# lrjconan/LanczosNetwork

Measured on NVIDIA H100. Metric: QM8 molecules/sec (forward), higher is better.
Workload: dtype f32

## Files before the change

### lanczosnetwork_b200/csrc/sm90.cuh

```cuda
#pragma once
#include <cuda.h>
#include <cuda_runtime.h>
#include <stdint.h>

namespace sm90 {

__device__ __forceinline__ uint32_t smem_u32(const void* p) {
  return static_cast<uint32_t>(__cvta_generic_to_shared(p));
}

__device__ __forceinline__ void mbar_init(uint64_t* bar, uint32_t count) {
  asm volatile("mbarrier.init.shared::cta.b64 [%0], %1;" ::"r"(smem_u32(bar)), "r"(count));
}
__device__ __forceinline__ void fence_barrier_init() {
  asm volatile("fence.mbarrier_init.release.cluster;" ::: "memory");
}
__device__ __forceinline__ void mbar_arrive(uint64_t* bar) {
  asm volatile("mbarrier.arrive.shared::cta.b64 _, [%0];" ::"r"(smem_u32(bar)) : "memory");
}
__device__ __forceinline__ void mbar_arrive_expect_tx(uint64_t* bar, uint32_t bytes) {
  asm volatile("mbarrier.arrive.expect_tx.shared::cta.b64 _, [%0], %1;" ::"r"(smem_u32(bar)),
               "r"(bytes)
               : "memory");
}
__device__ __forceinline__ bool mbar_try_wait(uint64_t* bar, uint32_t parity) {
  uint32_t ok;
  asm volatile(
      "{\n\t.reg .pred p;\n\t"
      "mbarrier.try_wait.parity.shared::cta.b64 p, [%1], %2;\n\t"
      "selp.b32 %0, 1, 0, p;\n\t}"
      : "=r"(ok)
      : "r"(smem_u32(bar)), "r"(parity)
      : "memory");
  return ok != 0;
}
__device__ __forceinline__ void mbar_wait(uint64_t* bar, uint32_t parity) {
  while (!mbar_try_wait(bar, parity)) {
  }
}

__device__ __forceinline__ void tma_prefetch_desc(const CUtensorMap* m) {
  asm volatile("prefetch.tensormap [%0];" ::"l"(reinterpret_cast<uint64_t>(m)) : "memory");
}
__device__ __forceinline__ void tma_load_2d(void* smem_dst, const CUtensorMap* m, uint64_t* bar,
                                            int32_t c0, int32_t c1) {
  asm volatile(
      "cp.async.bulk.tensor.2d.shared::cluster.global.mbarrier::complete_tx::bytes"
      " [%0], [%1, {%3, %4}], [%2];"
      ::"r"(smem_u32(smem_dst)), "l"(reinterpret_cast<uint64_t>(m)), "r"(smem_u32(bar)), "r"(c0),
      "r"(c1)
      : "memory");
}

__device__ __forceinline__ void cp_async_16(void* smem_dst, const void* gmem_src) {
  asm volatile("cp.async.cg.shared.global [%0], [%1], 16;" ::"r"(smem_u32(smem_dst)), "l"(gmem_src)
               : "memory");
}
__device__ __forceinline__ void cp_async_4(void* smem_dst, const void* gmem_src) {
  asm volatile("cp.async.ca.shared.global [%0], [%1], 4;" ::"r"(smem_u32(smem_dst)), "l"(gmem_src)
               : "memory");
}
__device__ __forceinline__ void cp_async_wait_all() {
  asm volatile("cp.async.commit_group;\n\tcp.async.wait_group 0;" ::: "memory");
}

__device__ __forceinline__ void fence_proxy_async() {
  asm volatile("fence.proxy.async.shared::cta;" ::: "memory");
}

__device__ __forceinline__ bool elect_one() {
  uint32_t pred;
  asm volatile(
      "{\n\t.reg .pred p;\n\t"
      "elect.sync _|p, 0xffffffff;\n\t"
      "selp.b32 %0, 1, 0, p;\n\t}"
      : "=r"(pred));
  return pred != 0;
}

__device__ __forceinline__ uint32_t tf32_rna_bits(float v) {
  uint32_t r;
  asm("cvt.rna.tf32.f32 %0, %1;" : "=r"(r) : "f"(v));
  return r;
}

__device__ __forceinline__ uint64_t wgmma_desc_kmajor_sw128(uint32_t smem_addr) {
  uint64_t d = 0;
  d |= (uint64_t)((smem_addr >> 4) & 0x3FFFu);
  d |= (uint64_t)1 << 16;
  d |= (uint64_t)64 << 32;
  d |= (uint64_t)1 << 62;
  return d;
}
__device__ __forceinline__ void wgmma_fence() { asm volatile("wgmma.fence.sync.aligned;" ::: "memory"); }
__device__ __forceinline__ void wgmma_commit() { asm volatile("wgmma.commit_group.sync.aligned;" ::: "memory"); }
__device__ __forceinline__ void wgmma_wait_all() { asm volatile("wgmma.wait_group.sync.aligned 0;" ::: "memory"); }


__device__ __forceinline__ void wgmma_n128(float (&d)[128], uint64_t a_desc, uint64_t b_desc, uint32_t scale_d) {
  asm volatile(
      "{\n\t.reg .pred p;\n\t"
      "setp.ne.b32 p, %66, 0;\n\t"
      "wgmma.mma_async.sync.aligned.m64n128k8.f32.tf32.tf32 "
      "{"
      "%0, %1, %2, %3, %4, %5, %6, %7, %8, %9, %10, %11, %12, %13, %14, %15, "
      "%16, %17, %18, %19, %20, %21, %22, %23, %24, %25, %26, %27, %28, %29, %30, %31, "
      "%32, %33, %34, %35, %36, %37, %38, %39, %40, %41, %42, %43, %44, %45, %46, %47, "
      "%48, %49, %50, %51, %52, %53, %54, %55, %56, %57, %58, %59, %60, %61, %62, %63"
      "}, %64, %65, p, 1, 1;\n\t}"
      : "+f"(d[0]), "+f"(d[1]), "+f"(d[2]), "+f"(d[3]), "+f"(d[4]), "+f"(d[5]), "+f"(d[6]), "+f"(d[7]),
        "+f"(d[8]), "+f"(d[9]), "+f"(d[10]), "+f"(d[11]), "+f"(d[12]), "+f"(d[13]), "+f"(d[14]), "+f"(d[15]),
        "+f"(d[16]), "+f"(d[17]), "+f"(d[18]), "+f"(d[19]), "+f"(d[20]), "+f"(d[21]), "+f"(d[22]), "+f"(d[23]),
        "+f"(d[24]), "+f"(d[25]), "+f"(d[26]), "+f"(d[27]), "+f"(d[28]), "+f"(d[29]), "+f"(d[30]), "+f"(d[31]),
        "+f"(d[32]), "+f"(d[33]), "+f"(d[34]), "+f"(d[35]), "+f"(d[36]), "+f"(d[37]), "+f"(d[38]), "+f"(d[39]),
        "+f"(d[40]), "+f"(d[41]), "+f"(d[42]), "+f"(d[43]), "+f"(d[44]), "+f"(d[45]), "+f"(d[46]), "+f"(d[47]),
        "+f"(d[48]), "+f"(d[49]), "+f"(d[50]), "+f"(d[51]), "+f"(d[52]), "+f"(d[53]), "+f"(d[54]), "+f"(d[55]),
        "+f"(d[56]), "+f"(d[57]), "+f"(d[58]), "+f"(d[59]), "+f"(d[60]), "+f"(d[61]), "+f"(d[62]), "+f"(d[63])
      : "l"(a_desc), "l"(b_desc), "r"(scale_d));
}

__device__ __forceinline__ void wgmma_n128_hi(float (&d)[128], uint64_t a_desc, uint64_t b_desc, uint32_t scale_d) {
  asm volatile(
      "{\n\t.reg .pred p;\n\t"
      "setp.ne.b32 p, %66, 0;\n\t"
      "wgmma.mma_async.sync.aligned.m64n128k8.f32.tf32.tf32 "
      "{"
      "%0, %1, %2, %3, %4, %5, %6, %7, %8, %9, %10, %11, %12, %13, %14, %15, "
      "%16, %17, %18, %19, %20, %21, %22, %23, %24, %25, %26, %27, %28, %29, %30, %31, "
      "%32, %33, %34, %35, %36, %37, %38, %39, %40, %41, %42, %43, %44, %45, %46, %47, "
      "%48, %49, %50, %51, %52, %53, %54, %55, %56, %57, %58, %59, %60, %61, %62, %63"
      "}, %64, %65, p, 1, 1;\n\t}"
      : "+f"(d[64]), "+f"(d[65]), "+f"(d[66]), "+f"(d[67]), "+f"(d[68]), "+f"(d[69]), "+f"(d[70]), "+f"(d[71]),
        "+f"(d[72]), "+f"(d[73]), "+f"(d[74]), "+f"(d[75]), "+f"(d[76]), "+f"(d[77]), "+f"(d[78]), "+f"(d[79]),
        "+f"(d[80]), "+f"(d[81]), "+f"(d[82]), "+f"(d[83]), "+f"(d[84]), "+f"(d[85]), "+f"(d[86]), "+f"(d[87]),
        "+f"(d[88]), "+f"(d[89]), "+f"(d[90]), "+f"(d[91]), "+f"(d[92]), "+f"(d[93]), "+f"(d[94]), "+f"(d[95]),
        "+f"(d[96]), "+f"(d[97]), "+f"(d[98]), "+f"(d[99]), "+f"(d[100]), "+f"(d[101]), "+f"(d[102]), "+f"(d[103]),
        "+f"(d[104]), "+f"(d[105]), "+f"(d[106]), "+f"(d[107]), "+f"(d[108]), "+f"(d[109]), "+f"(d[110]), "+f"(d[111]),
        "+f"(d[112]), "+f"(d[113]), "+f"(d[114]), "+f"(d[115]), "+f"(d[116]), "+f"(d[117]), "+f"(d[118]), "+f"(d[119]),
        "+f"(d[120]), "+f"(d[121]), "+f"(d[122]), "+f"(d[123]), "+f"(d[124]), "+f"(d[125]), "+f"(d[126]), "+f"(d[127])
      : "l"(a_desc), "l"(b_desc), "r"(scale_d));
}

}
```

### lanczosnetwork_b200/csrc/tc_gemm.cuh

```cuda
#pragma once
#include "common.cuh"
#include "sm90.cuh"
#include <stdlib.h>
#include <type_traits>

namespace tcg {

constexpr int BM = 128, BN = 128, BK = 32;
constexpr int NGROUPS = 1;
constexpr int TILE_B_BYTES = BN * BK * 4;
constexpr int STAGE_B_BYTES = 2 * TILE_B_BYTES;
constexpr int TILE_A_BYTES = BM * BK * 4;
constexpr int STAGE_A_BYTES = 2 * TILE_A_BYTES;
constexpr int EW = 16;
constexpr int PRODUCER_THREADS = 128 * NGROUPS;
constexpr int CONSUMER_WARP0 = PRODUCER_THREADS / 32;
constexpr int CONSUMER_THREADS = 256;
constexpr int THREADS = PRODUCER_THREADS + CONSUMER_THREADS;
constexpr int MAX_B_STAGES = 6, MAX_A_STAGES = 4;
__host__ __device__ constexpr int core_smem(int stages_b, int stages_a) {
  return stages_b * STAGE_B_BYTES + stages_a * STAGE_A_BYTES + 256;
}
__host__ __device__ constexpr int pass_cols(int stages_a) {
  return stages_a * STAGE_A_BYTES / (BM * 4) < BN ? stages_a * STAGE_A_BYTES / (BM * 4) : BN;
}

__device__ __forceinline__ uint8_t* a_ring(uint8_t* policy_smem, int stages_b, int stages_a) {
  return policy_smem - core_smem(stages_b, stages_a) + stages_b * STAGE_B_BYTES;
}

struct Core {
  uint8_t* Bst;
  uint8_t* Ast;
  uint64_t* b_full;
  uint64_t* b_empty;
  uint64_t* a_full;
  uint64_t* a_empty;
  uint64_t* stg_full;
  uint64_t* stg_empty;
  uint64_t* kept_read;
};

__device__ __forceinline__ Core carve(uint8_t* base, int stages_b, int stages_a) {
  Core c;
  c.Bst = base;
  c.Ast = base + stages_b * STAGE_B_BYTES;
  uint64_t* bars = reinterpret_cast<uint64_t*>(c.Ast + stages_a * STAGE_A_BYTES);
  c.b_full = bars;
  c.b_empty = c.b_full + MAX_B_STAGES;
  c.a_full = c.b_empty + MAX_B_STAGES;
  c.a_empty = c.a_full + MAX_A_STAGES;
  c.stg_full = c.a_empty + MAX_A_STAGES;
  c.stg_empty = c.stg_full + 1;
  c.kept_read = c.stg_empty + 1;
  return c;
}

__device__ unsigned long long* g_prof = nullptr;

struct PhaseTimer {
  unsigned long long* buf;
  long long t0;
  __device__ __forceinline__ void start(int cta, int tid) {
    buf = (tid == 0 && g_prof) ? g_prof + cta * 32 : nullptr;
    if (buf) t0 = clock64();
  }
  __device__ __forceinline__ void start_if(int cta, bool owner) {
    buf = (owner && g_prof) ? g_prof + cta * 32 : nullptr;
    if (buf) t0 = clock64();
  }
  __device__ __forceinline__ void lap(int slot) {
    if (buf) { long long t = clock64(); atomicAdd(&buf[slot], (unsigned long long)(t - t0)); t0 = t; }
  }
};

__device__ __forceinline__ void producers_sync() {
  asm volatile("bar.sync 1, %0;" ::"n"(PRODUCER_THREADS) : "memory");
}
__device__ __forceinline__ void consumers_sync() {
  asm volatile("bar.sync 2, %0;" ::"n"(CONSUMER_THREADS) : "memory");
}

__device__ __forceinline__ int stg_index(int row, int col, int pw) {
  return row * pw + ((((col >> 2) ^ row) & (pw / 4 - 1)) << 2) + (col & 3);
}

template <class P, class = void> struct HasAccInit : std::false_type {};
template <class P> struct HasAccInit<P, std::void_t<decltype(&P::acc_init)>> : std::true_type {};
template <class P, class = void> struct HasOperandFromAcc : std::false_type {};
template <class P> struct HasOperandFromAcc<P, std::void_t<decltype(&P::operand_from_acc)>> : std::true_type {};

template <class Policy>
__device__ __forceinline__ bool next_from_acc(const typename Policy::Params& p, int cta, int ncta, int it,
                                              int nsteps, int& nkb_next) {
  if (it + 1 >= nsteps) return false;
  int m_tile, sub;
  Policy::decode(p, cta, ncta, it + 1, m_tile, sub);
  nkb_next = Policy::num_kblocks(p, sub);
  return Policy::operand_from_acc(p, sub);
}

template <class Policy>
__global__ void __launch_bounds__(THREADS, 1)
tc_gemm_kernel(const __grid_constant__ CUtensorMap map_hi,
               const __grid_constant__ CUtensorMap map_lo, const typename Policy::Params p) {
  extern __shared__ __align__(16) uint8_t smem_raw[];
  const uint32_t pad = (1024u - (sm90::smem_u32(smem_raw) & 1023u)) & 1023u;
  uint8_t* base = smem_raw + pad;
  constexpr int SB = Policy::kStagesB, SA = Policy::kStagesA;
  static_assert(SB >= 1 && SB <= MAX_B_STAGES && SA >= 1 && SA <= MAX_A_STAGES, "ring depths");
  constexpr int PW = pass_cols(SA);
  constexpr int NPASS = BN / PW;
  constexpr bool kAccInit = HasAccInit<Policy>::value;
  static_assert(!kAccInit || NPASS == 1, "a drain kept in the A ring must fit it in one pass");
  constexpr bool kOpAcc = HasOperandFromAcc<Policy>::value;
  static_assert(!kOpAcc || SA * BK >= BN, "an operand written from the accumulators needs one A stage per k-block");
  Core c = carve(base, SB, SA);
  uint8_t* policy_smem = base + core_smem(SB, SA);
  float* stg = reinterpret_cast<float*>(c.Ast);

  const int tid = threadIdx.x, warp = tid >> 5, lane = tid & 31;
  const int cta = blockIdx.x, ncta = gridDim.x;
  const int nsteps = Policy::num_steps(p, cta, ncta);
  unsigned long long prof_ns0 = 0;
  long long prof_c0 = 0;
  if (tid == 0 && g_prof) {
    asm volatile("mov.u64 %0, %globaltimer;" : "=l"(prof_ns0));
    prof_c0 = clock64();
  }

  if (warp == CONSUMER_WARP0 && lane == 0) {
    sm90::tma_prefetch_desc(&map_hi);
    sm90::tma_prefetch_desc(&map_lo);
    for (int s = 0; s < SB; ++s) {
      sm90::mbar_init(&c.b_full[s], 1);
      sm90::mbar_init(&c.b_empty[s], CONSUMER_THREADS / 32);
    }
    for (int s = 0; s < SA; ++s) {
      sm90::mbar_init(&c.a_full[s], PRODUCER_THREADS);
      sm90::mbar_init(&c.a_empty[s], CONSUMER_THREADS / 32);
    }
    sm90::mbar_init(c.stg_full, CONSUMER_THREADS);
    sm90::mbar_init(c.stg_empty, PRODUCER_THREADS);
    sm90::mbar_init(c.kept_read, CONSUMER_THREADS / 32);
    sm90::fence_barrier_init();
  }
  __syncthreads();

  if (warp < CONSUMER_WARP0) {
    const int r = tid & 127;
    Policy pol(p, policy_smem, tid);
    uint32_t cnt = 0;
    uint32_t npass = 0;
    uint32_t nkept = 0;
    bool after_kept = false;
    for (int it = 0; it < nsteps; ++it) {
      int m_tile, sub;
      Policy::decode(p, cta, ncta, it, m_tile, sub);
      int nkb = Policy::num_kblocks(p, sub);
      bool kept = false, to_acc = false;
      if constexpr (kAccInit) kept = Policy::drain_kept(p, sub);
      if constexpr (kOpAcc) {
        if (Policy::operand_from_acc(p, sub)) nkb = 0;
        int nkb_next;
        to_acc = next_from_acc<Policy>(p, cta, ncta, it, nsteps, nkb_next);
      }
      PhaseTimer tm;
      tm.start(cta, tid);
      pol.step_begin(m_tile, sub, 0, tm);
      for (int kb = 0; kb < nkb; ++kb, ++cnt) {
        float v[32];
        if (!(p.dbg & 8)) pol.produce(sub, kb, v);
        const uint32_t sa = cnt % SA;
        if (kAccInit && kb == 0 && after_kept) {
          sm90::mbar_wait(c.kept_read, nkept & 1u);
          ++nkept;
        }
        sm90::mbar_wait(&c.a_empty[sa], ((cnt / SA) & 1u) ^ 1u);
        if (!(p.dbg & 1)) {
          uint8_t* hi = c.Ast + sa * STAGE_A_BYTES + r * 128;
#pragma unroll
          for (int j = 0; j < 8; ++j) {
            uint4 h, l;
            h.x = sm90::tf32_rna_bits(v[4 * j + 0]); h.y = sm90::tf32_rna_bits(v[4 * j + 1]);
            h.z = sm90::tf32_rna_bits(v[4 * j + 2]); h.w = sm90::tf32_rna_bits(v[4 * j + 3]);
            l.x = sm90::tf32_rna_bits(v[4 * j + 0] - __uint_as_float(h.x));
            l.y = sm90::tf32_rna_bits(v[4 * j + 1] - __uint_as_float(h.y));
            l.z = sm90::tf32_rna_bits(v[4 * j + 2] - __uint_as_float(h.z));
            l.w = sm90::tf32_rna_bits(v[4 * j + 3] - __uint_as_float(h.w));
            const int off = (j ^ (r & 7)) * 16;
            *reinterpret_cast<uint4*>(hi + off) = h;
            *reinterpret_cast<uint4*>(hi + TILE_A_BYTES + off) = l;
          }
        }
        sm90::fence_proxy_async();
        sm90::mbar_arrive(&c.a_full[sa]);
      }
      tm.lap((sub & 1) ? 8 : 3);
      pol.pre_epilogue(sub);
      tm.lap(4);
#pragma unroll 1
      for (int q = 0; q < (kept || to_acc ? 0 : NPASS); ++q, ++npass) {
        sm90::mbar_wait(c.stg_full, npass & 1u);
        if (q == 0) tm.lap((sub & 1) ? 9 : 5);
#pragma unroll 1
        for (int col = q * PW; col < (q + 1) * PW; col += EW) {
          float x[EW];
#pragma unroll
          for (int j = 0; j < EW; j += 4) {
            const float4 t = *reinterpret_cast<const float4*>(stg + stg_index(r, col - q * PW + j, PW));
            x[j] = t.x; x[j + 1] = t.y; x[j + 2] = t.z; x[j + 3] = t.w;
          }
          pol.store(sub, col, x);
        }
        sm90::mbar_arrive(c.stg_empty);
      }
      tm.lap(7);
      producers_sync();
      pol.post_epilogue(sub);
      tm.lap(10);
      after_kept = kept;
    }
  } else {
    const int wg = (warp - CONSUMER_WARP0) >> 2;
    const int wq = warp & 3;
    float d[128];
    uint32_t cnt = 0, npass = 0;
    uint32_t nacc = 0;
    bool after_kept = false;
    const int row0 = wg * 64 + wq * 16 + (lane >> 2), cl = 2 * (lane & 3);
    const bool issuer = warp == CONSUMER_WARP0;
    int l_it = 0, l_kb = 0, l_nkb = -1, l_sub = 0;
    uint32_t l_cnt = 0;
    auto load_next = [&]() {
      while (l_it < nsteps) {
        if (l_nkb < 0) {
          int mt;
          Policy::decode(p, cta, ncta, l_it, mt, l_sub);
          l_nkb = Policy::num_kblocks(p, l_sub);
        }
        if (l_kb < l_nkb) break;
        ++l_it; l_kb = 0; l_nkb = -1;
      }
      if (l_it >= nsteps) return;
      int col0, row0;
      Policy::w_coords(p, l_sub, l_kb, col0, row0);
      const uint32_t st = l_cnt % SB;
      sm90::mbar_wait(&c.b_empty[st], ((l_cnt / SB) & 1u) ^ 1u);
      if (sm90::elect_one()) {
        if (p.dbg & 4) {
          sm90::mbar_arrive(&c.b_full[st]);
        } else {
          uint8_t* dst = c.Bst + st * STAGE_B_BYTES;
          sm90::mbar_arrive_expect_tx(&c.b_full[st], STAGE_B_BYTES);
          sm90::tma_load_2d(dst, &map_hi, &c.b_full[st], col0, row0);
          sm90::tma_load_2d(dst + TILE_B_BYTES, &map_lo, &c.b_full[st], col0, row0);
        }
      }
      __syncwarp();
      ++l_kb; ++l_cnt;
    };
    if (issuer)
      for (int i = 0; i < SB; ++i) load_next();
    for (int it = 0; it < nsteps; ++it) {
      int m_tile, sub;
      Policy::decode(p, cta, ncta, it, m_tile, sub);
      const int nkb = Policy::num_kblocks(p, sub);
      bool kept = false, from_acc = false, to_acc = false;
      int nkb_next = 0;
      if constexpr (kOpAcc) {
        from_acc = Policy::operand_from_acc(p, sub);
        to_acc = next_from_acc<Policy>(p, cta, ncta, it, nsteps, nkb_next);
      }
      if constexpr (kAccInit) {
        kept = Policy::drain_kept(p, sub);
        if (!Policy::acc_init(p, policy_smem, stg, sub, row0, cl, d)) {
#pragma unroll
          for (int i = 0; i < 128; ++i) d[i] = 0.f;
        }
        if (after_kept) {
          __syncwarp();
          if (lane == 0) sm90::mbar_arrive(c.kept_read);
        }
      } else {
#pragma unroll
        for (int i = 0; i < 128; ++i) d[i] = 0.f;
      }
      for (int kb = 0; kb < nkb; ++kb, ++cnt) {
        const uint32_t acnt = cnt - nacc;
        const uint32_t sb = cnt % SB, sa = from_acc ? (uint32_t)kb : acnt % SA;
        sm90::mbar_wait(&c.b_full[sb], (cnt / SB) & 1u);
        if (!from_acc) sm90::mbar_wait(&c.a_full[sa], (acnt / SA) & 1u);
        if (!(p.dbg & 2)) {
          const uint32_t a_hi = sm90::smem_u32(c.Ast + sa * STAGE_A_BYTES) + wg * 64 * 128;
          const uint32_t a_lo = a_hi + TILE_A_BYTES;
          const uint32_t b = sm90::smem_u32(c.Bst + sb * STAGE_B_BYTES);
          sm90::wgmma_fence();
#pragma unroll
          for (int k = 0; k < BK / 8; ++k) {
            const uint64_t ah = sm90::wgmma_desc_kmajor_sw128(a_hi + 32 * k);
            const uint64_t wh = sm90::wgmma_desc_kmajor_sw128(b + 32 * k);
            sm90::wgmma_n128(d, ah, wh, 1u);
            sm90::wgmma_n128_hi(d, ah, sm90::wgmma_desc_kmajor_sw128(b + TILE_B_BYTES + 32 * k), 1u);
            sm90::wgmma_n128_hi(d, sm90::wgmma_desc_kmajor_sw128(a_lo + 32 * k), wh, 1u);
          }
          sm90::wgmma_commit();
          sm90::wgmma_wait_all();
        }
        __syncwarp();
        if (lane == 0) {
          if (!from_acc) sm90::mbar_arrive(&c.a_empty[sa]);
          sm90::mbar_arrive(&c.b_empty[sb]);
        }
        if (issuer) load_next();
      }
      if (from_acc) nacc += nkb;
      PhaseTimer ctm;
      if (to_acc) ctm.start_if(cta, tid == PRODUCER_THREADS);
      consumers_sync();
      if (to_acc) {
        if constexpr (kOpAcc) {
#pragma unroll
          for (int i = 0; i < 64; i += 2) {
            const int col = 8 * (i / 4) + cl, row = row0 + 8 * ((i / 2) % 2), kb = i / 16;
            if (kb < nkb_next) {
              const float y0 = Policy::acc_operand(p, policy_smem, sub, col, d[i] + d[i + 64]);
              const float y1 = Policy::acc_operand(p, policy_smem, sub, col + 1, d[i + 1] + d[i + 65]);
              uint2 h, l;
              h.x = sm90::tf32_rna_bits(y0); h.y = sm90::tf32_rna_bits(y1);
              l.x = sm90::tf32_rna_bits(y0 - __uint_as_float(h.x));
              l.y = sm90::tf32_rna_bits(y1 - __uint_as_float(h.y));
              uint8_t* dst = c.Ast + kb * STAGE_A_BYTES + row * 128 + (((((col & 31) >> 2) ^ row) & 7) << 4) +
                             (col & 3) * 4;
              *reinterpret_cast<uint2*>(dst) = h;
              *reinterpret_cast<uint2*>(dst + TILE_A_BYTES) = l;
            }
          }
          sm90::fence_proxy_async();
          consumers_sync();
          ctm.lap(14);
        }
      } else {
#pragma unroll
        for (int q = 0; q < NPASS; ++q, npass += kept ? 0 : 1) {
          if (!kept) sm90::mbar_wait(c.stg_empty, (npass & 1u) ^ 1u);
#pragma unroll
          for (int i = 0; i < 64; i += 2) {
            const int col = 8 * (i / 4) + cl, row = row0 + 8 * ((i / 2) % 2);
            if (col >= q * PW && col < (q + 1) * PW)
              *reinterpret_cast<float2*>(stg + stg_index(row, col - q * PW, PW)) =
                  make_float2(d[i] + d[i + 64], d[i + 1] + d[i + 65]);
          }
          if (!kept) sm90::mbar_arrive(c.stg_full);
        }
      }
      if (kept) consumers_sync();
      after_kept = kept;
    }
  }

  __syncthreads();
  if (tid == 0 && g_prof) {
    unsigned long long ns1;
    asm volatile("mov.u64 %0, %globaltimer;" : "=l"(ns1));
    atomicAdd(&g_prof[cta * 32 + 11], ns1 - prof_ns0);
    atomicAdd(&g_prof[cta * 32 + 12], (unsigned long long)(clock64() - prof_c0));
    g_prof[cta * 32 + 13] = prof_ns0;
  }
}

__device__ __forceinline__ void store_row_chunk(float* orow, int ncols, const float* bias, bool relu,
                                                int col, const float (&x)[EW]) {
  if (orow == nullptr || col >= ncols) return;
  const bool vec_ok = (reinterpret_cast<uintptr_t>(orow + col) & 15) == 0;
#pragma unroll
  for (int j = 0; j < EW; j += 4) {
    float o[4];
#pragma unroll
    for (int u = 0; u < 4; ++u) {
      const int n = col + j + u;
      float y = x[j + u];
      if (n < ncols) {
        if (bias) y += __ldg(bias + n);
        if (relu) y = fmaxf(y, 0.f);
      }
      o[u] = y;
    }
    if (vec_ok && col + j + 3 < ncols) {
      *reinterpret_cast<float4*>(orow + col + j) = make_float4(o[0], o[1], o[2], o[3]);
    } else {
#pragma unroll
      for (int u = 0; u < 4; ++u)
        if (col + j + u < ncols) orow[col + j + u] = o[u];
    }
  }
}

typedef CUresult (*EncodeTiledFn)(CUtensorMap*, CUtensorMapDataType, cuuint32_t, void*,
                                  const cuuint64_t*, const cuuint64_t*, const cuuint32_t*,
                                  const cuuint32_t*, CUtensorMapInterleave, CUtensorMapSwizzle,
                                  CUtensorMapL2promotion, CUtensorMapFloatOOBfill);

inline EncodeTiledFn get_encode_fn() {
  static EncodeTiledFn fn = nullptr;
  if (!fn) {
    void* ptr = nullptr;
    cudaDriverEntryPointQueryResult q;
    if (cudaGetDriverEntryPoint("cuTensorMapEncodeTiled", &ptr, cudaEnableDefault, &q) == cudaSuccess &&
        q == cudaDriverEntryPointSuccess)
      fn = reinterpret_cast<EncodeTiledFn>(ptr);
  }
  return fn;
}

inline int make_weight_map(CUtensorMap* map, const float* W, int rows, int cols, const char* who,
                           int box_rows = BN) {
  EncodeTiledFn enc = get_encode_fn();
  if (!enc) { lnb::set_err("%s: cuTensorMapEncodeTiled unavailable", who); return LNB_ERR_UNSUPPORTED; }
  cuuint64_t gdim[2] = {(cuuint64_t)cols, (cuuint64_t)rows};
  cuuint64_t gstride[1] = {(cuuint64_t)cols * sizeof(float)};
  cuuint32_t box[2] = {(cuuint32_t)BK, (cuuint32_t)box_rows};
  cuuint32_t estr[2] = {1, 1};
  CUresult r = enc(map, CU_TENSOR_MAP_DATA_TYPE_FLOAT32, 2, const_cast<float*>(W), gdim, gstride,
                   box, estr, CU_TENSOR_MAP_INTERLEAVE_NONE, CU_TENSOR_MAP_SWIZZLE_128B,
                   CU_TENSOR_MAP_L2_PROMOTION_L2_256B, CU_TENSOR_MAP_FLOAT_OOB_FILL_NONE);
  if (r != CUDA_SUCCESS) {
    lnb::set_err("%s: cuTensorMapEncodeTiled failed (CUresult %d)", who, (int)r);
    return LNB_ERR_ARG;
  }
  return LNB_OK;
}

inline int debug_flags() {
  const char* e = getenv("LNB_DBG");
  return e ? atoi(e) : 0;
}

inline int sm_count() {
  int dev = 0, n = 132;
  if (cudaGetDevice(&dev) == cudaSuccess)
    cudaDeviceGetAttribute(&n, cudaDevAttrMultiProcessorCount, dev);
  return n > 0 ? n : 132;
}

static unsigned long long* g_prof_mirrored = nullptr;

static int sync_prof_buffer(const char* who) {
  unsigned long long* buf = lnb::prof_buffer();
  if (buf == g_prof_mirrored) return LNB_OK;
  cudaError_t e = cudaMemcpyToSymbol(g_prof, &buf, sizeof(buf));
  if (e != cudaSuccess) { lnb::set_err("%s: %s", who, cudaGetErrorString(e)); return (int)e; }
  g_prof_mirrored = buf;
  return LNB_OK;
}

template <class Pol>
static int launch(lnb_stream_t stream, const float* W_hi, const float* W_lo, int w_rows, int w_cols,
                  size_t smem, int items, const typename Pol::Params& p, const char* who) {
  CUtensorMap map_hi, map_lo;
  int rc = make_weight_map(&map_hi, W_hi, w_rows, w_cols, who);
  if (rc != LNB_OK) return rc;
  rc = make_weight_map(&map_lo, W_lo, w_rows, w_cols, who);
  if (rc != LNB_OK) return rc;
  rc = sync_prof_buffer(who);
  if (rc != LNB_OK) return rc;
  auto kern = tc_gemm_kernel<Pol>;
  cudaFuncSetAttribute(kern, cudaFuncAttributeMaxDynamicSharedMemorySize, (int)smem);
  const int grid = items < sm_count() ? items : sm_count();
  kern<<<grid, THREADS, smem, (cudaStream_t)stream>>>(map_hi, map_lo, p);
  lnb::count_launch();
  return lnb::finish_launch(who);
}

}
```

Measured before the change: 995,200.

## Keep one WGMMA group in flight and defer stage release in GEMM mainloop

When the policy does not initialise accumulators from a drain, the consumer loop now waits for only the previous wgmma group (wait_group 1) and releases the previous k-block's A/B stages, so tensor-core work on consecutive k-blocks can overlap. It also compiles the debug skip flags into template variants instead of testing them at runtime, makes role and step count warp-uniform via shuffles, and folds the TMA issue into one predicated, elected PTX block with uniform-branch barrier waits. The deferred release holds each stage one k-block longer, which can stall the TMA refill when the ring is shallow, and the operand fences may add register-pressure constraints.

Result: faster. 1.066 million, median of 6 (+7.1%).

```diff
diff --git a/lanczosnetwork_b200/csrc/sm90.cuh b/lanczosnetwork_b200/csrc/sm90.cuh
--- a/lanczosnetwork_b200/csrc/sm90.cuh
+++ b/lanczosnetwork_b200/csrc/sm90.cuh
@@ -39,6 +39,26 @@
   }
 }
 
+__device__ __forceinline__ void mbar_wait_uniform(uint64_t* bar, uint32_t parity) {
+  asm volatile(
+      "{\n\t.reg .pred p;\n\t"
+      "LAB_WAIT:\n\t"
+      "mbarrier.try_wait.parity.shared::cta.b64 p, [%0], %1;\n\t"
+      "@p bra DONE;\n\t"
+      "bra.uni LAB_WAIT;\n\t"
+      "DONE:\n\t}"
+      ::"r"(smem_u32(bar)), "r"(parity)
+      : "memory");
+}
+__device__ __forceinline__ void mbar_arrive_pred(uint64_t* bar, bool pred) {
+  asm volatile(
+      "{\n\t.reg .pred p;\n\t"
+      "setp.ne.b32 p, %1, 0;\n\t"
+      "@p mbarrier.arrive.shared::cta.b64 _, [%0];\n\t}"
+      ::"r"(smem_u32(bar)), "r"((uint32_t)pred)
+      : "memory");
+}
+
 __device__ __forceinline__ void tma_prefetch_desc(const CUtensorMap* m) {
   asm volatile("prefetch.tensormap [%0];" ::"l"(reinterpret_cast<uint64_t>(m)) : "memory");
 }
@@ -68,6 +88,35 @@
   asm volatile("fence.proxy.async.shared::cta;" ::: "memory");
 }
 
+template <bool skip_load = false>
+__device__ __forceinline__ void tma_load_2d_pair_elected(bool pred, uint64_t* bar, uint32_t bytes, void* dst0,
+                                                         const CUtensorMap* m0, void* dst1, const CUtensorMap* m1,
+                                                         int32_t c0, int32_t c1) {
+  if constexpr (skip_load) {
+    asm volatile(
+        "{\n\t.reg .pred e, p;\n\t"
+        "elect.sync _|e, 0xffffffff;\n\t"
+        "setp.ne.and.b32 p, %1, 0, e;\n\t"
+        "@p mbarrier.arrive.shared::cta.b64 _, [%0];\n\t}"
+        ::"r"(smem_u32(bar)), "r"((uint32_t)pred)
+        : "memory");
+  } else {
+    asm volatile(
+        "{\n\t.reg .pred e, p;\n\t"
+        "elect.sync _|e, 0xffffffff;\n\t"
+        "setp.ne.and.b32 p, %1, 0, e;\n\t"
+        "@p mbarrier.arrive.expect_tx.shared::cta.b64 _, [%0], %2;\n\t"
+        "@p cp.async.bulk.tensor.2d.shared::cluster.global.mbarrier::complete_tx::bytes"
+        " [%3], [%4, {%7, %8}], [%0];\n\t"
+        "@p cp.async.bulk.tensor.2d.shared::cluster.global.mbarrier::complete_tx::bytes"
+        " [%5], [%6, {%7, %8}], [%0];\n\t}"
+        ::"r"(smem_u32(bar)), "r"((uint32_t)pred), "r"(bytes), "r"(smem_u32(dst0)),
+          "l"(reinterpret_cast<uint64_t>(m0)), "r"(smem_u32(dst1)), "l"(reinterpret_cast<uint64_t>(m1)),
+          "r"(c0), "r"(c1)
+        : "memory");
+  }
+}
+
 __device__ __forceinline__ bool elect_one() {
   uint32_t pred;
   asm volatile(
@@ -95,6 +144,11 @@
 __device__ __forceinline__ void wgmma_fence() { asm volatile("wgmma.fence.sync.aligned;" ::: "memory"); }
 __device__ __forceinline__ void wgmma_commit() { asm volatile("wgmma.commit_group.sync.aligned;" ::: "memory"); }
 __device__ __forceinline__ void wgmma_wait_all() { asm volatile("wgmma.wait_group.sync.aligned 0;" ::: "memory"); }
+__device__ __forceinline__ void wgmma_fence_operand(float (&d)[128]) {
+#pragma unroll
+  for (int i = 0; i < 128; ++i) asm volatile("" : "+f"(d[i])::"memory");
+}
+__device__ __forceinline__ void wgmma_wait_one() { asm volatile("wgmma.wait_group.sync.aligned 1;" ::: "memory"); }
 
 
 __device__ __forceinline__ void wgmma_n128(float (&d)[128], uint64_t a_desc, uint64_t b_desc, uint32_t scale_d) {
diff --git a/lanczosnetwork_b200/csrc/tc_gemm.cuh b/lanczosnetwork_b200/csrc/tc_gemm.cuh
--- a/lanczosnetwork_b200/csrc/tc_gemm.cuh
+++ b/lanczosnetwork_b200/csrc/tc_gemm.cuh
@@ -100,10 +100,12 @@
   return Policy::operand_from_acc(p, sub);
 }
 
-template <class Policy>
-__global__ void __launch_bounds__(THREADS, 1)
-tc_gemm_kernel(const __grid_constant__ CUtensorMap map_hi,
-               const __grid_constant__ CUtensorMap map_lo, const typename Policy::Params p) {
+constexpr int SKIP_MMA = 2;
+constexpr int SKIP_TMA = 4;
+
+template <class Policy, int kSkip>
+__device__ __forceinline__ void tc_gemm_body(const CUtensorMap& map_hi, const CUtensorMap& map_lo,
+                                             const typename Policy::Params& p) {
   extern __shared__ __align__(16) uint8_t smem_raw[];
   const uint32_t pad = (1024u - (sm90::smem_u32(smem_raw) & 1023u)) & 1023u;
   uint8_t* base = smem_raw + pad;
@@ -114,14 +116,16 @@
   constexpr bool kAccInit = HasAccInit<Policy>::value;
   static_assert(!kAccInit || NPASS == 1, "a drain kept in the A ring must fit it in one pass");
   constexpr bool kOpAcc = HasOperandFromAcc<Policy>::value;
+  constexpr bool kQueue = !kAccInit;
   static_assert(!kOpAcc || SA * BK >= BN, "an operand written from the accumulators needs one A stage per k-block");
   Core c = carve(base, SB, SA);
   uint8_t* policy_smem = base + core_smem(SB, SA);
   float* stg = reinterpret_cast<float*>(c.Ast);
 
   const int tid = threadIdx.x, warp = tid >> 5, lane = tid & 31;
+  const int role = __shfl_sync(0xffffffffu, tid / 128, 0);
   const int cta = blockIdx.x, ncta = gridDim.x;
-  const int nsteps = Policy::num_steps(p, cta, ncta);
+  const int nsteps = __shfl_sync(0xffffffffu, Policy::num_steps(p, cta, ncta), 0);
   unsigned long long prof_ns0 = 0;
   long long prof_c0 = 0;
   if (tid == 0 && g_prof) {
@@ -147,7 +151,7 @@
   }
   __syncthreads();
 
-  if (warp < CONSUMER_WARP0) {
+  if (role == 0) {
     const int r = tid & 127;
     Policy pol(p, policy_smem, tid);
     uint32_t cnt = 0;
@@ -222,14 +226,14 @@
       after_kept = kept;
     }
   } else {
-    const int wg = (warp - CONSUMER_WARP0) >> 2;
+    const int wg = role - 1;
     const int wq = warp & 3;
     float d[128];
     uint32_t cnt = 0, npass = 0;
     uint32_t nacc = 0;
     bool after_kept = false;
     const int row0 = wg * 64 + wq * 16 + (lane >> 2), cl = 2 * (lane & 3);
-    const bool issuer = warp == CONSUMER_WARP0;
+    const bool w_issuer = warp == CONSUMER_WARP0;
     int l_it = 0, l_kb = 0, l_nkb = -1, l_sub = 0;
     uint32_t l_cnt = 0;
     auto load_next = [&]() {
@@ -246,22 +250,18 @@
       int col0, row0;
       Policy::w_coords(p, l_sub, l_kb, col0, row0);
       const uint32_t st = l_cnt % SB;
-      sm90::mbar_wait(&c.b_empty[st], ((l_cnt / SB) & 1u) ^ 1u);
-      if (sm90::elect_one()) {
-        if (p.dbg & 4) {
-          sm90::mbar_arrive(&c.b_full[st]);
-        } else {
-          uint8_t* dst = c.Bst + st * STAGE_B_BYTES;
-          sm90::mbar_arrive_expect_tx(&c.b_full[st], STAGE_B_BYTES);
-          sm90::tma_load_2d(dst, &map_hi, &c.b_full[st], col0, row0);
-          sm90::tma_load_2d(dst + TILE_B_BYTES, &map_lo, &c.b_full[st], col0, row0);
-        }
-      }
-      __syncwarp();
+      sm90::mbar_wait_uniform(&c.b_empty[st], ((l_cnt / SB) & 1u) ^ 1u);
+      uint8_t* dst = c.Bst + st * STAGE_B_BYTES;
+      sm90::tma_load_2d_pair_elected<(kSkip & SKIP_TMA) != 0>(w_issuer, &c.b_full[st], STAGE_B_BYTES, dst, &map_hi,
+                                                               dst + TILE_B_BYTES, &map_lo, col0, row0);
       ++l_kb; ++l_cnt;
     };
-    if (issuer)
-      for (int i = 0; i < SB; ++i) load_next();
+    auto release = [&](uint32_t sb_rel, bool a_stage, uint32_t sa_rel) {
+      sm90::mbar_arrive_pred(&c.a_empty[sa_rel], a_stage && lane == 0);
+      sm90::mbar_arrive_pred(&c.b_empty[sb_rel], lane == 0);
+      load_next();
+    };
+    for (int i = 0; i < SB; ++i) load_next();
     for (int it = 0; it < nsteps; ++it) {
       int m_tile, sub;
       Policy::decode(p, cta, ncta, it, m_tile, sub);
@@ -274,6 +274,7 @@
       }
       if constexpr (kAccInit) {
         kept = Policy::drain_kept(p, sub);
+        sm90::wgmma_fence_operand(d);
         if (!Policy::acc_init(p, policy_smem, stg, sub, row0, cl, d)) {
 #pragma unroll
           for (int i = 0; i < 128; ++i) d[i] = 0.f;
@@ -286,15 +287,17 @@
 #pragma unroll
         for (int i = 0; i < 128; ++i) d[i] = 0.f;
       }
+      sm90::wgmma_fence_operand(d);
       for (int kb = 0; kb < nkb; ++kb, ++cnt) {
         const uint32_t acnt = cnt - nacc;
         const uint32_t sb = cnt % SB, sa = from_acc ? (uint32_t)kb : acnt % SA;
-        sm90::mbar_wait(&c.b_full[sb], (cnt / SB) & 1u);
-        if (!from_acc) sm90::mbar_wait(&c.a_full[sa], (acnt / SA) & 1u);
-        if (!(p.dbg & 2)) {
+        sm90::mbar_wait_uniform(&c.b_full[sb], (cnt / SB) & 1u);
+        if (!from_acc) sm90::mbar_wait_uniform(&c.a_full[sa], (acnt / SA) & 1u);
+        if constexpr (!(kSkip & SKIP_MMA)) {
           const uint32_t a_hi = sm90::smem_u32(c.Ast + sa * STAGE_A_BYTES) + wg * 64 * 128;
           const uint32_t a_lo = a_hi + TILE_A_BYTES;
           const uint32_t b = sm90::smem_u32(c.Bst + sb * STAGE_B_BYTES);
+          sm90::wgmma_fence_operand(d);
           sm90::wgmma_fence();
 #pragma unroll
           for (int k = 0; k < BK / 8; ++k) {
@@ -305,15 +308,22 @@
             sm90::wgmma_n128_hi(d, sm90::wgmma_desc_kmajor_sw128(a_lo + 32 * k), wh, 1u);
           }
           sm90::wgmma_commit();
-          sm90::wgmma_wait_all();
-        }
-        __syncwarp();
-        if (lane == 0) {
-          if (!from_acc) sm90::mbar_arrive(&c.a_empty[sa]);
-          sm90::mbar_arrive(&c.b_empty[sb]);
-        }
-        if (issuer) load_next();
-      }
+          if constexpr (kQueue) sm90::wgmma_wait_one();
+          else sm90::wgmma_wait_all();
+          sm90::wgmma_fence_operand(d);
+        }
+        if constexpr (kQueue) {
+          if (kb > 0) release((cnt - 1) % SB, !from_acc, from_acc ? (uint32_t)(kb - 1) : (acnt - 1) % SA);
+        } else {
+          release(sb, !from_acc, sa);
+        }
+      }
+      if constexpr (!(kSkip & SKIP_MMA)) {
+        sm90::wgmma_wait_all();
+        sm90::wgmma_fence_operand(d);
+      }
+      if (kQueue && nkb > 0)
+        release((cnt - 1) % SB, !from_acc, from_acc ? (uint32_t)(nkb - 1) : (cnt - nacc - 1) % SA);
       if (from_acc) nacc += nkb;
       PhaseTimer ctm;
       if (to_acc) ctm.start_if(cta, tid == PRODUCER_THREADS);
@@ -369,6 +379,20 @@
   }
 }
 
+template <class Policy>
+__global__ void __launch_bounds__(THREADS, 1)
+tc_gemm_kernel(const __grid_constant__ CUtensorMap map_hi,
+               const __grid_constant__ CUtensorMap map_lo, const typename Policy::Params p) {
+  tc_gemm_body<Policy, 0>(map_hi, map_lo, p);
+}
+
+template <class Policy, int kSkip>
+__global__ void __launch_bounds__(THREADS, 1)
+tc_gemm_probe_kernel(const __grid_constant__ CUtensorMap map_hi,
+                     const __grid_constant__ CUtensorMap map_lo, const typename Policy::Params p) {
+  tc_gemm_body<Policy, kSkip>(map_hi, map_lo, p);
+}
+
 __device__ __forceinline__ void store_row_chunk(float* orow, int ncols, const float* bias, bool relu,
                                                 int col, const float (&x)[EW]) {
   if (orow == nullptr || col >= ncols) return;
@@ -464,7 +488,11 @@
   if (rc != LNB_OK) return rc;
   rc = sync_prof_buffer(who);
   if (rc != LNB_OK) return rc;
-  auto kern = tc_gemm_kernel<Pol>;
+  const int skip = p.dbg & (SKIP_MMA | SKIP_TMA);
+  auto kern = skip == 0                    ? tc_gemm_kernel<Pol>
+              : skip == SKIP_MMA           ? tc_gemm_probe_kernel<Pol, SKIP_MMA>
+              : skip == SKIP_TMA           ? tc_gemm_probe_kernel<Pol, SKIP_TMA>
+                                           : tc_gemm_probe_kernel<Pol, SKIP_MMA | SKIP_TMA>;
   cudaFuncSetAttribute(kern, cudaFuncAttributeMaxDynamicSharedMemorySize, (int)smem);
   const int grid = items < sm_count() ? items : sm_count();
   kern<<<grid, THREADS, smem, (cudaStream_t)stream>>>(map_hi, map_lo, p);
```
